# DannielSilva/MM-VQA

Measured on AMD Instinct MI355X. Metric: samples/sec ROCO-MLM pretrain (resnet152+transformer, bs16/GPU, 224^2, seq32), higher is better.
Workload: dtype f32; 1 GPU; pretrain/roco_train.py MLM-only: resnet152 + transformer(4 layers, 12 heads), num_vis 5, hidden 768, vocab 30522, per-GPU batch 16, 224x224, T=32; fwd + log_softmax/NLL + bwd + grad all-reduce + Adam; dropout on, train-mode BN; random-init weights; global_batch=16, seq_len=32, parallelism=dp1

## Files before the change

mm-vqa_amd/csrc/igemm.hip:

```cpp
#include <string>
#include <type_traits>
#include <vector>

#include "kernels.h"

struct FastDiv {
  uint32_t mul, shr, d;
};
struct GemmAux {
  FastDiv ohw, ow;
  int fast;
  int stagger;
  float* part;
  int ldsc;
  int pad0;
  int sk_gx, sk_gy;
  int sk_slots;
  float* sk_part;
  unsigned* sk_cnt;
  int tick;
  int xcd;
};

__device__ __forceinline__ int fdiv(int n, const FastDiv& f) {
// ... 202 lines not shown
          for (int j = 0; j < 4; ++j) {
            double* d = red + (c4 * 4 + j) * 3;
            atomicAdd(d, (double)sa[j]);
            atomicAdd(d + 1, (double)sb[j]);
            if (st2) atomicAdd(d + 2, (double)sc[j]);
          }
        }
        if (colsum) {
#pragma unroll
          for (int j = 0; j < 4; ++j) atomicAdd(&redf[c4 * 4 + j], cs[j]);
        }
      }
      __syncthreads();
      TRACE_EPI(2);
      if (tid < BN && n0 + tid < N) {
        if (st1) {
          const double* d = red + tid * 3;
          const int slot = slot_seed & ((p.stat_slots > 0 ? p.stat_slots : MMVQA_STAT_SLOTS) - 1);
          double* d1 = st1 + ((size_t)slot * N + n0 + tid) * 2;
          atomicAdd(d1, d[0]);
          atomicAdd(d1 + 1, d[1]);
          if (st2) {
            double* d2 = st2 + ((size_t)slot * N + n0 + tid) * 2;
            atomicAdd(d2, d[0]);
            atomicAdd(d2 + 1, d[2]);
          }
        }
        if (colsum) atomicAdd(&colsum[n0 + tid], redf[tid]);
      }
    }
    }
}

template <int BM, int BN, int BK, int KIND, bool NCHW, int KS, int PREC = MMVQA_PREC_F32>
__global__ __launch_bounds__(256 * KS, 2) void igemm_kernel(const GemmParams p, const GemmAux x) {
  constexpr int NT = 256 * KS;
  constexpr int WM = BM / 2, WN = BN / 2, TM = WM / 32, TN = WN / 32;
  constexpr bool F16 = (PREC == MMVQA_PREC_F16);
  static_assert(!F16 || KS == 1, "the f16 family has no 8-wave form");
  constexpr bool PIPE = TM * TN <= 2;
  constexpr int LDK = F16 ? BK + 8 : BK + 4;
  constexpr int KQ = BK / 4;
  constexpr int RSTEP = NT / KQ;
  constexpr int NA = BM / RSTEP, NB = BN / RSTEP;
  constexpr bool A_ROWK = (KIND != KIND_WGRAD);
  constexpr bool B_ROWK = (KIND == KIND_FWD);
  constexpr int LDA_KM = F16 ? km_ld_h(BM) : BM + 4, LDB_KM = F16 ? km_ld_h(BN) : BN + 4;
  constexpr int A_TILE = A_ROWK ? tile_rowk<PREC>(BM, BK) : tile_km<PREC>(BM, BK);
  constexpr int B_TILE = B_ROWK ? tile_rowk<PREC>(BN, BK) : tile_km<PREC>(BN, BK);
  constexpr int A_X4 = BM / 4, A_KSTEP = NT / A_X4, NA_KM = BK / A_KSTEP;
  constexpr int B_X4 = BN / 4, B_KSTEP = NT / B_X4, NB_KM = BK / B_KSTEP;
  constexpr int NAC = A_ROWK ? NA : NA_KM;
  constexpr int NBC = B_ROWK ? NB : NB_KM;

  TRACE_MARK(0);
  TRACE_STALL_DECL
  extern __shared__ __attribute__((aligned(16))) float smem[];
  float* As = smem;
  float* Bs = smem + 2 * A_TILE;
  int* taptab = reinterpret_cast<int*>(smem + 2 * A_TILE + 2 * B_TILE);
  float* ctab = smem + 2 * A_TILE + 2 * B_TILE + MAX_TAPS;

  const int nkt_total = (p.K + BK - 1) / BK;
  __shared__ int sk_last;
  const int tid = threadIdx.x;
  const int lane = tid & 63, wave = (tid >> 6) & 3, ks = tid >> 8;
  const int li = lane & 31, lh = lane >> 5;
  const int wm0 = (wave >> 1) * WM, wn0 = (wave & 1) * WN;
// ... 174 lines not shown
      int tap = 0;
      if (taps > 1) { tap = nn / p.g_Cs; b_kh = tap / p.g_KW; b_kw = tap - b_kh * p.g_KW; }
      b_ci = nn - tap * p.g_Cs;
      if (p.b_pro != PRO_NONE && b_colvalid) { bc0 = ld4(p.b_c0 + b_ci); bc1 = ld4(p.b_c1 + b_ci); }
    } else {
#pragma unroll
      for (int j = 0; j < 4; ++j) {
        int kk = nn + j;
        int tap = kk / p.g_Cs;
        b_cc[j] = kk - tap * p.g_Cs;
        b_dy[j] = tap / p.g_KW; b_dx[j] = tap - b_dy[j] * p.g_KW;
        if (kk >= p.N) b_dy[j] = -(1 << 24);
      }
    }
#pragma unroll
    for (int r = 0; r < NB_KM; ++r) { b_base[r] = k_begin + bkm_k0 + B_KSTEP * r; b_ok0[r] = 1; }
  }

  struct Stage {
    f32x4 ra[NAC], ra2[NAC], rb[NBC], rb2[NBC];
    uint32_t a_ok, b_ok;
    f32x4 ac0, ac1, ac2;
    int tm[NAC];
    int pm[NBC], tmb[NBC];
  };

  f32x16 acc[TM][TN];
#pragma unroll
  for (int i = 0; i < TM; ++i)
#pragma unroll
    for (int j = 0; j < TN; ++j)
#pragma unroll
      for (int e = 0; e < 16; ++e) acc[i][j][e] = 0.f;

  const int adv_tap = BK / p.g_Cs, adv_c = BK - adv_tap * p.g_Cs;

  auto lds_put = [&](float* tile, int e, f32x4 v) __attribute__((always_inline)) {
    if constexpr (F16) *reinterpret_cast<f16x4*>(reinterpret_cast<_Float16*>(tile) + e) = __builtin_convertvector(v, f16x4);
    else *reinterpret_cast<f32x4*>(&tile[e]) = v;
  };

  auto run = [&](auto APRO_T, auto BPRO_T, auto FAST_T, auto LDSC_T) __attribute__((always_inline)) {
    constexpr int APRO = decltype(APRO_T)::value;
    constexpr int BPRO = decltype(BPRO_T)::value;
    constexpr int FAST = decltype(FAST_T)::value;
    constexpr bool LDSC = decltype(LDSC_T)::value;
    constexpr bool A_TWO = (APRO == PRO_DZ);
    constexpr bool A_AFF = (APRO == PRO_AFFINE_RELU || APRO == PRO_AFFINE_SILU || APRO == PRO_SILU_GATE);
    constexpr bool B_AFF = (BPRO == PRO_AFFINE_RELU || BPRO == PRO_AFFINE_SILU || BPRO == PRO_SILU_GATE);

    constexpr int NLP = 1 + NAC + NBC;
    bool lt_kvalid = false;
    int lt_toff = 0;
    int lt_kh[4], lt_kw[4], lt_c[4];
    auto load_piece = [&](Stage& S, int kt, int i) __attribute__((always_inline)) {
      if (i == 0) {
        S.a_ok = 0; S.b_ok = 0;
        if constexpr (A_ROWK && !NCHW) {
          lt_kvalid = a_tap < taps;
          lt_toff = taptab[lt_kvalid ? a_tap : 0];
          if constexpr (A_AFF || A_TWO) {
            const int cc = lt_kvalid ? a_c : 0;
            S.ac0 = ld4(p.a_c0 + cc); S.ac1 = ld4(p.a_c1 + cc);
            if constexpr (APRO == PRO_DZ) S.ac2 = ld4(p.a_c2 + cc);
          }
        }
// ... 332 lines not shown
        }
      } else {
        const int r = c - NAC;
        f32x4 v = S.rb[r];
        if constexpr (KIND == KIND_WGRAD && BPRO == PRO_AFFINE_RELU) {
          const f32x2 lo = __builtin_elementwise_fma(v.xy, bc0.xy, bc1.xy), hi = __builtin_elementwise_fma(v.zw, bc0.zw, bc1.zw);
          if constexpr (FAST == 2) {
            const float lim = __builtin_bit_cast(float, S.tmb[r] & 0x7f800000);
            v[0] = __builtin_amdgcn_fmed3f(lo[0], 0.f, lim); v[1] = __builtin_amdgcn_fmed3f(lo[1], 0.f, lim);
            v[2] = __builtin_amdgcn_fmed3f(hi[0], 0.f, lim); v[3] = __builtin_amdgcn_fmed3f(hi[1], 0.f, lim);
          } else {
            v[0] = fmaxf(lo[0], 0.f); v[1] = fmaxf(lo[1], 0.f); v[2] = fmaxf(hi[0], 0.f); v[3] = fmaxf(hi[1], 0.f);
          }
        }
        if constexpr (B_ROWK) {
          lds_put(bs, (b_r0 + RSTEP * r) * LDK + b_kq, v);
        } else {
          lds_put(bs, (bkm_k0 + B_KSTEP * r) * LDB_KM + bkm_x4 * 4, v);
        }
      }
    };
    auto LP = [&](Stage& S, int kt, int i) __attribute__((always_inline)) {
      if constexpr (FAST != 0) fload_piece(S, i); else load_piece(S, kt, i);
    };
    auto SC = [&](Stage& S, int buf, int kt, int c) __attribute__((always_inline)) {
      if constexpr (FAST != 0) fstore_chunk(S, buf, c); else store_chunk(S, buf, kt, c);
    };
    auto LT = [&](Stage& S, int kt) __attribute__((always_inline)) {
#pragma unroll
      for (int i = 0; i < NLP; ++i) LP(S, kt, i);
    };

    auto read_frags = [&](const float* as, const float* bs, int kg, f32x4 (&fa)[TM], f32x4 (&fb)[TN]) __attribute__((always_inline)) {
#pragma unroll
      for (int i = 0; i < TM; ++i) {
        if constexpr (A_ROWK) {
          fa[i] = *reinterpret_cast<const f32x4*>(&as[(wm0 + i * 32 + li) * LDK + kg * 8 + lh * 4]);
        } else {
#pragma unroll
          for (int j = 0; j < 4; ++j) fa[i][j] = as[(kg * 8 + lh * 4 + j) * LDA_KM + wm0 + i * 32 + li];
        }
      }
#pragma unroll
      for (int i = 0; i < TN; ++i) {
        if constexpr (B_ROWK) {
          fb[i] = *reinterpret_cast<const f32x4*>(&bs[(wn0 + i * 32 + li) * LDK + kg * 8 + lh * 4]);
        } else {
#pragma unroll
          for (int j = 0; j < 4; ++j) fb[i][j] = bs[(kg * 8 + lh * 4 + j) * LDB_KM + wn0 + i * 32 + li];
        }
      }
    };

    constexpr int NC = NAC + NBC;
    constexpr int NKG = BK / 8 / KS;

    TRACE_MARK(1);
    Stage S0, S1;
    S0.a_ok = S0.b_ok = S1.a_ok = S1.b_ok = 0;
    S0.ac0 = S1.ac0 = ac0_i; S0.ac1 = S1.ac1 = ac1_i; S0.ac2 = S1.ac2 = ac2_i;

    if constexpr (FAST == 2 && KIND == KIND_WGRAD) {
#pragma unroll
      for (int r = 0; r < NBC; ++r) { S0.pm[r] = tload(f_voffT[r], 0); S1.pm[r] = tload(f_voffT[r], BK * 4); }
    }
    if (nkt > 0) {
      LT(S0, kt_begin);
      if constexpr (PIPE) LT(S1, kt_begin + 1);
#pragma unroll
      for (int c = 0; c < NC; ++c) SC(S0, 0, kt_begin, c);
      if constexpr (FAST != 0 && PIPE && !F16) f_halo(S0);
    }
    __builtin_amdgcn_s_waitcnt(0x0F70);
    __syncthreads();
    TRACE_MARK(2);

    if constexpr (F16) {
      auto frag = [&](const float* tile, int rowk, int ldkm, int r0, int st) __attribute__((always_inline)) {
        const _Float16* t = reinterpret_cast<const _Float16*>(tile);
        if (rowk) return *reinterpret_cast<const f16x8*>(t + (r0 + li) * LDK + st * 16 + lh * 8);
        const int g = lane >> 4, q = (lane >> 2) & 3, pp = lane & 3;
        const _Float16* b = t + (st * 16 + (g >> 1) * 8 + q) * ldkm + r0 + (g & 1) * 16 + 4 * pp;
        typedef __attribute__((address_space(3))) s16x4 lds_s16x4;
        const f16x4 lo = __builtin_bit_cast(f16x4, __builtin_amdgcn_ds_read_tr16_b64_v4i16((lds_s16x4*)(b)));
        const f16x4 hi = __builtin_bit_cast(f16x4, __builtin_amdgcn_ds_read_tr16_b64_v4i16((lds_s16x4*)(b + 4 * ldkm)));
        return __builtin_shufflevector(lo, hi, 0, 1, 2, 3, 4, 5, 6, 7);
      };
      auto body16 = [&](int t, Stage& Sload, Stage& Sstore) __attribute__((always_inline)) {
        const int buf = t & 1;
        LT(Sload, kt_begin + t + (PIPE ? 2 : 1));
        const float* as = As + buf * A_TILE;
        const float* bs = Bs + buf * B_TILE;
#pragma unroll
        for (int st = 0; st < BK / 16; ++st) {
          f16x8 fa[TM], fb[TN];
#pragma unroll
          for (int i = 0; i < TM; ++i) fa[i] = frag(as, A_ROWK, LDA_KM, wm0 + i * 32, st);
#pragma unroll
          for (int i = 0; i < TN; ++i) fb[i] = frag(bs, B_ROWK, LDB_KM, wn0 + i * 32, st);
#pragma unroll
          for (int a = 0; a < TM; ++a)
#pragma unroll
            for (int b = 0; b < TN; ++b)
              acc[a][b] = __builtin_amdgcn_mfma_f32_32x32x16_f16(fa[a], fb[b], acc[a][b], 0, 0, 0);
        }
#pragma unroll
        for (int c = 0; c < NC; ++c) SC(Sstore, buf ^ 1, kt_begin + t + 1, c);
        __syncthreads();
      };
      if constexpr (PIPE) {
        int t = 0;
        for (; t + 1 < nkt; t += 2) {
          body16(t, S0, S1);
          body16(t + 1, S1, S0);
        }
        if (t < nkt) body16(t, S0, S1);
      } else {
        for (int t = 0; t < nkt; ++t) body16(t, S0, S0);
      }
    } else if constexpr (PIPE) {
      f32x4 fa[2][TM], fb[2][TN];
      read_frags(As, Bs, ks, fa[0], fb[0]);
      constexpr int MPG = 4 * TM * TN;
      constexpr int NS = NKG * MPG;
      constexpr int SB = NS - MPG;
      constexpr int L0 = 1;
      constexpr int LSTR = (NS - 2) / NLP > 0 ? (NS - 2) / NLP : 1;
      constexpr int ST0 = LSTR >= 2 ? L0 + 1 : L0 + NLP;
      constexpr int STR = LSTR >= 2 ? LSTR : ((SB - ST0) / NC > 0 ? (SB - ST0) / NC : 1);
      static_assert(ST0 + (NC - 1) * STR < SB, "load/store pieces do not fit in front of the barrier");
      constexpr int SV = SB - (NS >= 32 ? 5 : 3);
      constexpr int FLS = (SV - 2) / NC > 0 ? (SV - 2) / NC : 1;
      static_assert(2 + (NC - 1) * FLS < SV, "fast load slots must precede the VALU slot");
      static_assert(2 + (NC - 1) * FLS + 1 < NS, "staggered group: advance/halo slot inside the K-tile");
      auto body = [&](auto STG_T, int t, Stage& Sload, Stage& Sstore) __attribute__((always_inline)) {
        constexpr bool STG = decltype(STG_T)::value;
        constexpr int SVX = STG ? 1 : SV;
        const int buf = t & 1;
        const float* as = As + buf * A_TILE;
        const float* bs = Bs + buf * B_TILE;
        static_for<NS>([&](auto SI) __attribute__((always_inline)) {
          constexpr int sl = decltype(SI)::value, kk = sl / MPG, g = sl % MPG;
          constexpr int j = g / (TM * TN), ta = (g % (TM * TN)) / TN, tb = g % TN;
          if constexpr (g == 0) {
            if constexpr (kk + 1 < NKG) {
              read_frags(as, bs, (kk + 1) * KS + ks, fa[(kk + 1) & 1], fb[(kk + 1) & 1]);
            } else {
#ifdef IGEMM_TRACE
              {
                const unsigned long long ta = __builtin_readcyclecounter();
                __builtin_amdgcn_s_waitcnt(0xC07F);
                const unsigned long long tb = __builtin_readcyclecounter();
                __syncthreads();
                const unsigned long long tc = __builtin_readcyclecounter();
                tr_lgkm += tb - ta; tr_bar += tc - tb;
              }
#elif !defined(EXP_NOBAR)
              __syncthreads();
#endif
              read_frags(As + (buf ^ 1) * A_TILE, Bs + (buf ^ 1) * B_TILE, ks, fa[0], fb[0]);
            }
          }
          acc[ta][tb] = __builtin_amdgcn_mfma_f32_32x32x2f32(fa[kk & 1][ta][j], fb[kk & 1][tb][j], acc[ta][tb], 0, 0, 0);
#ifndef EXP_NOLOAD
          if constexpr (FAST != 0) {
            if constexpr (sl == 1) f_scalars(Sload);
            if constexpr (sl >= 2 && (STG || sl < SV) && (sl - 2) % FLS == 0 && (sl - 2) / FLS < NC) f_chunk(Sload, (sl - 2) / FLS);
          } else {
            if constexpr (sl >= L0 && (sl - L0) % LSTR == 0 && (sl - L0) / LSTR < NLP)
              LP(Sload, kt_begin + t + 2, (sl - L0) / LSTR);
          }
#endif
#ifndef EXP_NOSTORE
#ifdef IGEMM_TRACE
          if constexpr (sl == SVX && FAST != 0) {
            constexpr int NLD = (A_ROWK && (A_AFF || A_TWO) ? (APRO == PRO_DZ ? 3 : 2) : 0) + NAC * (A_TWO ? 2 : 1) + NBC;
            const unsigned long long ta = __builtin_readcyclecounter();
            __builtin_amdgcn_s_waitcnt(0x0F70 | (NLD & 15) | ((NLD >> 4) << 14));
            const unsigned long long tb = __builtin_readcyclecounter();
            tr_vm += tb - ta;
          }
#endif
          if constexpr (FAST != 0) {
            if constexpr (sl == SVX) {
#pragma unroll
              for (int c = 0; c < NC; ++c) fstore_chunk(Sstore, buf ^ 1, c);
              if constexpr (!STG) {
                f_advance();
                f_halo(Sstore);
              }
            }
            if constexpr (STG && sl == 2 + (NC - 1) * FLS + 1) {
              f_advance();
              f_halo(Sstore);
            }
          } else {
// ... 68 lines not shown
      } else {
        switch (p.a_pro) {
          case PRO_AFFINE_RELU: run(I1{}, I0{}, G{}, L0{}); break;
          case PRO_AFFINE_SILU: run(I4{}, I0{}, G{}, L0{}); break;
          case PRO_SILU_GATE: run(I5{}, I0{}, G{}, L0{}); break;
          default: run(I0{}, I0{}, G{}, L0{});
        }
      }
    } else if constexpr (KIND == KIND_DGRAD) {
      if (x.fast == 1) {
        if (p.a_pro == PRO_DZ) { if (x.ldsc) run(I2{}, I0{}, F1{}, L1{}); else run(I2{}, I0{}, F1{}, L0{}); }
        else run(I0{}, I0{}, F1{}, L0{});
      } else if (x.fast == 2) {
        if (p.a_pro == PRO_DZ) { if (x.ldsc) run(I2{}, I0{}, F2{}, L1{}); else run(I2{}, I0{}, F2{}, L0{}); }
        else run(I0{}, I0{}, F2{}, L0{});
      } else {
        if (p.a_pro == PRO_DZ) run(I2{}, I0{}, G{}, L0{}); else run(I0{}, I0{}, G{}, L0{});
      }
    } else {
      if (x.fast == 1) {
        if (p.a_pro == PRO_DZ) {
          if (p.b_pro == PRO_AFFINE_RELU) run(I2{}, I1{}, F1{}, L0{}); else run(I2{}, I0{}, F1{}, L0{});
        } else {
          if (p.b_pro == PRO_AFFINE_RELU) run(I0{}, I1{}, F1{}, L0{}); else run(I0{}, I0{}, F1{}, L0{});
        }
      } else if (x.fast == 2) {
        if constexpr (TM * TN == 1) {
          if (p.a_pro == PRO_DZ) {
            if (p.b_pro == PRO_AFFINE_RELU) run(I2{}, I1{}, F2{}, L0{}); else run(I2{}, I0{}, F2{}, L0{});
          } else {
            if (p.b_pro == PRO_AFFINE_RELU) run(I0{}, I1{}, F2{}, L0{}); else run(I0{}, I0{}, F2{}, L0{});
          }
        }
      } else if (p.a_pro == PRO_DZ) {
        switch (p.b_pro) {
          case PRO_AFFINE_RELU: run(I2{}, I1{}, G{}, L0{}); break;
          case PRO_AFFINE_SILU: run(I2{}, I4{}, G{}, L0{}); break;
          case PRO_SILU_GATE: run(I2{}, I5{}, G{}, L0{}); break;
          default: run(I2{}, I0{}, G{}, L0{});
        }
      } else {
        switch (p.b_pro) {
          case PRO_AFFINE_RELU: run(I0{}, I1{}, G{}, L0{}); break;
          case PRO_AFFINE_SILU: run(I0{}, I4{}, G{}, L0{}); break;
          case PRO_SILU_GATE: run(I0{}, I5{}, G{}, L0{}); break;
          default: run(I0{}, I0{}, G{}, L0{});
        }
      }
    }
  }

  TRACE_MARK(3);
  TRACE_STALL_FLUSH();
  constexpr int LDC = BN + 4;
  constexpr int CH = BN / 4;
  constexpr int RP = NT / CH;
  constexpr int NPASS = BM / RP;
  float* ctile = smem;
  if (KS == 1 || ks == 0) {
    static_for<TM * TN * 16>([&](auto I) {
      constexpr int i = decltype(I)::value;
      constexpr int a = i / (TN * 16), b = (i / 16) % TN, e = i % 16;
      ctile[(wm0 + a * 32 + (e & 3) + 8 * (e >> 2) + 4 * lh) * LDC + wn0 + b * 32 + li] = acc[a][b][e];
    });
  }
  __syncthreads();
  if constexpr (KS > 1) {
    if (ks == 1) {
      static_for<TM * TN * 16>([&](auto I) {
        constexpr int i = decltype(I)::value;
        constexpr int a = i / (TN * 16), b = (i / 16) % TN, e = i % 16;
        ctile[(wm0 + a * 32 + (e & 3) + 8 * (e >> 2) + 4 * lh) * LDC + wn0 + b * 32 + li] += acc[a][b][e];
      });
    }
    __syncthreads();
  }

  TRACE_EPI(0);
  const int M = p.M, N = p.N;
  const int c4 = tid % CH, rg = tid / CH;
  const int col = n0 + c4 * 4;
  const bool full = col + 3 < N;
  auto ldv = [&](const float* base, size_t off) __attribute__((always_inline)) {
    f32x4 r = {0, 0, 0, 0};
    if (full && !(off & 3)) r = ld4(base + off);
    else {
#pragma unroll
      for (int j = 0; j < 4; ++j) if (col + j < N) r[j] = base[off + j];
    }
    return r;
  };
  auto stv = [&](float* base, size_t off, f32x4 v) __attribute__((always_inline)) {
    if (full && !(off & 3)) *reinterpret_cast<f32x4*>(base + off) = v;
    else {
#pragma unroll
      for (int j = 0; j < 4; ++j) if (col + j < N) base[off + j] = v[j];
    }
  };

  if (x.tick != 0) {
// ... 150 lines not shown
                                    const size_t off = (size_t)row * N + col;
                                    if (col + 3 < N && !(off & 3)) {
                                      f32x4 t[SK_MAX];
#pragma unroll
                                      for (int s = 0; s < SK_MAX; ++s)
                                        t[s] = s < nsplit ? ld4(part + s * MN + off) : f32x4{0, 0, 0, 0};
#pragma unroll
                                      for (int s = 0; s < SK_MAX; ++s) v += t[s];
                                    } else {
                                      for (int s = 0; s < nsplit; ++s)
#pragma unroll
                                        for (int j = 0; j < 4; ++j)
                                          if (col + j < N) v[j] += part[s * MN + off + j];
                                    }
                                  }
                                  return v;
                                });
}

static FastDiv make_fastdiv(int d) {
  FastDiv f;
  f.d = (uint32_t)d;
  if (d <= 1) { f.mul = 0; f.shr = 0; f.d = 1; return f; }
  int lg = 31;
  while (lg > 0 && !((uint32_t)d >> lg)) --lg;
  if (d & (d - 1)) ++lg;
  const int pw = 31 + lg;
  const uint64_t m = ((1ull << pw) + (uint64_t)d - 1) / (uint64_t)d;
  f.mul = (uint32_t)m;
  f.shr = (uint32_t)(pw - 32);
  return f;
}

template <int BM, int BN, int BK, int KIND, bool NCHW, int KS = 1, int PREC = MMVQA_PREC_F32>
static int launch_cfg(GemmParams p, hipStream_t stream) {
  constexpr bool A_ROWK = (KIND != KIND_WGRAD);
  constexpr bool B_ROWK = (KIND == KIND_FWD);
  constexpr int A_TILE = A_ROWK ? tile_rowk<PREC>(BM, BK) : tile_km<PREC>(BM, BK);
  constexpr int B_TILE = B_ROWK ? tile_rowk<PREC>(BN, BK) : tile_km<PREC>(BN, BK);
  constexpr size_t tile_floats = (size_t)(2 * A_TILE + 2 * B_TILE + MAX_TAPS);
  constexpr size_t epi_floats = (size_t)BM * (BN + 4) + 8 * BN;
  constexpr size_t smem_max = (tile_floats + FOLD_MAX_FLOATS > epi_floats ? tile_floats + FOLD_MAX_FLOATS : epi_floats) * sizeof(float);
  static int attr_dev_mask = 0;
  int dev = 0;
  (void)hipGetDevice(&dev);
  if (!(attr_dev_mask >> (dev & 31) & 1)) {
    HIP_CHECK_RET(hipFuncSetAttribute((const void*)igemm_kernel<BM, BN, BK, KIND, NCHW, KS, PREC>,
                                      hipFuncAttributeMaxDynamicSharedMemorySize, (int)smem_max));
    attr_dev_mask |= 1 << (dev & 31);
  }
  GemmAux x;
  x.ohw = make_fastdiv(p.g_OH * p.g_OW);
  x.ow = make_fastdiv(p.g_OW);
  x.fast = 0;
  static const int stagger_on = getenv("MMVQA_IGEMM_NOSTAGGER") ? 0 : 1;
  x.stagger = stagger_on;
  x.part = (KIND != KIND_WGRAD && !NCHW && p.splitk > 1 && !p.c_atomic) ? p.sk_ws : nullptr;
  if (!NCHW && (p.K % BK == 0 || (KIND == KIND_WGRAD && p.pixmask)) && !p.gate && !getenv("MMVQA_IGEMM_GENERAL")) {
    const int taps = p.g_KH * p.g_KW;
    const double lim = 2147483648.0 - 16777216.0;
    if (KIND != KIND_WGRAD) {
      const bool pro_ok = (KIND == KIND_FWD) ? (p.a_pro == PRO_NONE || p.a_pro == PRO_AFFINE_RELU)
                                             : (p.a_pro == PRO_NONE || p.a_pro == PRO_DZ);
      const double a_bytes = (KIND == KIND_FWD) ? (double)p.M * p.g_stride * p.g_stride * p.a_ld * 4.0 + (double)(p.g_SW + 2) * p.g_KH * p.a_ld * 4.0
                                                : (double)p.M * p.a_ld * 4.0;
      const double b_bytes = (KIND == KIND_FWD) ? (double)p.N * p.b_ld * 4.0 : (double)p.g_Cs * p.b_ld * 4.0;
      if (pro_ok && p.b_pro == PRO_NONE && p.g_Cs % BK == 0 && p.g_stride <= 2 && a_bytes < lim && b_bytes < lim &&
          (KIND == KIND_FWD || p.N % 4 == 0))
        x.fast = (taps > 1 || (KIND == KIND_DGRAD && p.g_stride > 1)) ? 2 : 1;
    } else {
      const bool pro_ok = (p.a_pro == PRO_NONE || p.a_pro == PRO_DZ) && (p.b_pro == PRO_NONE || p.b_pro == PRO_AFFINE_RELU);
      if (pro_ok && taps == 1 && p.K % BK == 0 && p.g_stride == 1 && p.g_pad == 0 && p.M % 4 == 0 && p.N % 4 == 0 &&
          (double)p.K * p.a_ld * 4.0 < lim && (double)p.K * p.b_ld * 4.0 < lim)
        x.fast = 1;
      else if (pro_ok && taps > 1 && taps <= 32 && p.pixmask && p.g_stride == 1 && p.g_OH == p.g_SH && p.g_OW == p.g_SW &&
               2 * p.g_pad == p.g_KH - 1 && p.g_KH == p.g_KW && BM == 64 && BN == 64 && p.g_Cs % BN == 0 && p.M % 4 == 0 &&
               (double)p.K * p.a_ld * 4.0 < lim && (double)(p.K + (double)p.g_SW * p.g_KH) * p.b_ld * 4.0 < lim)
        x.fast = 2;
    }
  }
// ... 11 lines not shown
      const int C = A_ROWK ? p.g_Cs : p.M;
      if (!f.publish || !f.out0 || !f.out1 || !f.out2)
        return mmvqa_set_error(MMVQA_ERR_ARG, "igemm: this launch cannot fold its BatchNorm coefficients in the kernel and has nowhere to publish them");
      if (f.bwd)
        TRY_RET(k_bn_coef_bwd(stream, f.stat, C, f.count, f.gamma, f.mean, f.invstd, 1, f.out0, f.out1, f.out2, f.dgamma, f.dbeta));
      else
        TRY_RET(k_bn_coef_fwd_keep(stream, f.stat, C, f.count, f.eps, f.gamma, f.beta, f.run_mean, f.run_var, f.nbt, f.keep,
                                   f.reps, 1, f.out0, f.out1, f.out2, f.out3));
      p.a_c0 = f.out0; p.a_c1 = f.out1; p.a_c2 = f.out2;
      p.a_fold.stat = nullptr;
    }
  }
  const size_t smem = ((tile_floats + fold_floats > epi_floats ? tile_floats + fold_floats : epi_floats)) * sizeof(float);
  dim3 grid((p.N + BN - 1) / BN, (p.M + BM - 1) / BM, p.splitk);
  x.pad0 = 0; x.sk_gx = (int)grid.x; x.sk_gy = (int)grid.y; x.sk_slots = 0; x.sk_part = nullptr; x.sk_cnt = nullptr; x.tick = 0;
  static const bool finish_form = getenv("MMVQA_SK_FINISH") != nullptr;
  if (x.part && !finish_form && p.sk_cnt && p.splitk <= SK_PART_MAX && p.epi_mode == EPI_PLAIN) {
    const long long tiles = (long long)grid.x * grid.y;
    if (tiles <= p.sk_cnt_n && tiles * p.splitk * (long long)(BM * BN) <= p.sk_ws_floats) {
      x.tick = 1; x.part = nullptr; x.sk_slots = p.splitk; x.sk_part = p.sk_ws; x.sk_cnt = p.sk_cnt;
    }
  }
  static const int xcd_on = getenv("MMVQA_IGEMM_NOXCD") ? 0 : 1;
  const long nwg = (long)grid.x * grid.y * grid.z;
  x.xcd = 0;
  if (xcd_on && nwg >= 32 && !NCHW) {
    double a_bytes, b_bytes;
    if (KIND == KIND_WGRAD) { a_bytes = (double)p.K * p.M * (p.a_pro == PRO_DZ ? 2 : 1); b_bytes = (double)p.K * p.g_Cs; }
    else if (KIND == KIND_FWD) { a_bytes = (double)p.M * p.g_stride * p.g_stride * p.g_Cs; b_bytes = (double)p.N * p.K; }
    else { a_bytes = (double)p.M * p.g_Cs * (p.a_pro == PRO_DZ ? 2 : 1); b_bytes = (double)p.N * p.K; }
    x.xcd = (b_bytes > a_bytes && x.sk_gy > 1) ? 2 : (x.sk_gx > 1 ? 1 : 0);
  }
  if (getenv("MMVQA_IGEMM_LOG"))
    fprintf(stderr, "igemm kind %d fast %d tile %dx%dx%d ks %d M %d N %d K %d Cs %d taps %d stride %d apro %d bpro %d splitk %d fold %d tick %d prec %s\n", KIND, x.fast,
            BM, BN, BK, KS, p.M, p.N, p.K, p.g_Cs, p.g_KH * p.g_KW, p.g_stride, p.a_pro, p.b_pro, p.splitk, x.ldsc, x.tick,
            PREC == MMVQA_PREC_F16 ? "f16" : "f32");
  hipLaunchKernelGGL((igemm_kernel<BM, BN, BK, KIND, NCHW, KS, PREC>), grid, dim3(256 * KS), smem, stream, p, x);
  KERNEL_CHECK_RET();
  if (x.part) {
    hipLaunchKernelGGL(splitk_finish_kernel, dim3((p.N + 63) / 64, (p.M + 63) / 64), dim3(256), 0, stream, p, x.part,
                       p.splitk);
    KERNEL_CHECK_RET();
  }
  return MMVQA_OK;
}

static inline int cdiv(int a, int b) { return (a + b - 1) / b; }

static bool sk_eligible(const GemmParams& p, int kind) {
  return kind != KIND_WGRAD && p.sk_ws && p.sk_ws_floats > 0 && p.epi_mode == EPI_PLAIN && !p.c_atomic;
}

static thread_local IgemmTuner* g_tuner = nullptr;
void mmvqa_set_tuner(IgemmTuner* t) { g_tuner = t; }
static thread_local int g_prec = MMVQA_PREC_F32;
void mmvqa_set_igemm_precision(int prec) { g_prec = prec; }

static std::string tune_key(const GemmParams& p, int kind, int nchw) {
  char buf[176];
  snprintf(buf, sizeof(buf), "%d,%d,%d,%d,%d,%d,%d,%d,%d,%d,%d,%d,%d,%d,%d,%d", p.reserved0, kind, nchw, p.M, p.N, p.K,
           p.g_KH * p.g_KW, p.g_stride, p.g_Cs, p.a_pro, p.b_pro, p.epi_mode, p.act | (p.dact << 4),
           (p.stat1 ? 1 : 0) | (p.stat2 ? 2 : 0) | (p.Mk ? 4 : 0) | (p.R ? 8 : 0) | (p.Cpre ? 16 : 0) |
               (p.colsum ? 32 : 0) | (p.bias ? 64 : 0) | (p.sk_ws ? 128 : 0) | (p.a_fold.stat ? 256 : 0) | (p.sk_cnt ? 512 : 0),
           p.c_atomic, p.splitk);
  return buf;
}

static int launch_one(GemmParams p, int kind, int nchw, int tile, hipStream_t stream);

static int validate_desc(const GemmParams& p, int kind, int nchw) {
#define BAD(...) return mmvqa_set_error(MMVQA_ERR_ARG, "igemm: " __VA_ARGS__)
  if (kind < KIND_FWD || kind > KIND_WGRAD) BAD("unknown kind %d", kind);
  if (p.reserved0 != MMVQA_PREC_F32 && p.reserved0 != MMVQA_PREC_F16) BAD("unknown operand precision %d (reserved0)", p.reserved0);
  if (p.reserved1 != 0) BAD("reserved1=%d must be 0 (the persistent form was removed)", p.reserved1);
  if (p.reserved0 == MMVQA_PREC_F16 && (p.a_pro == PRO_AFFINE_SILU || p.a_pro == PRO_SILU_GATE || p.b_pro == PRO_AFFINE_SILU ||
                                        p.b_pro == PRO_SILU_GATE || p.gate))
    BAD("the f16 operand family has no SiLU / gate prologues (a_pro %d, b_pro %d)", p.a_pro, p.b_pro);
  if (!p.A || !p.B) BAD("operand pointer is null (A=%p B=%p)", (const void*)p.A, (const void*)p.B);
  if (!p.C && p.epi_mode != EPI_TAP_FWD) BAD("output pointer is null");
  const int KH = p.g_KH > 0 ? p.g_KH : 1, KW = p.g_KH > 0 ? p.g_KW : 1;
  const long taps = (long)KH * KW;
  if (KW <= 0 || p.g_Cs <= 0 || (p.g_KH > 0 && (p.g_stride <= 0 || p.g_pad < 0))) BAD("bad geometry (KH=%d KW=%d Cs=%d stride=%d pad=%d)", p.g_KH, p.g_KW, p.g_Cs, p.g_stride, p.g_pad);
  if (p.g_OH <= 0 || p.g_OW <= 0 || p.g_SH <= 0 || p.g_SW <= 0) BAD("bad image dims (SH=%d SW=%d OH=%d OW=%d)", p.g_SH, p.g_SW, p.g_OH, p.g_OW);
  const long ohw = (long)p.g_OH * p.g_OW;
  if (kind == KIND_WGRAD) {
    if ((long)p.N != taps * p.g_Cs) BAD("wgrad: N=%d != taps*Cs=%ld", p.N, taps * p.g_Cs);
    if (p.K % ohw) BAD("wgrad: K=%d is not a multiple of OH*OW=%ld", p.K, ohw);
    if (p.a_ld < p.M || (!nchw && p.b_ld < p.g_Cs) || p.c_ld < p.N) BAD("wgrad: leading dimension too small (a_ld=%d M=%d b_ld=%d Cs=%d c_ld=%d N=%d)", p.a_ld, p.M, p.b_ld, p.g_Cs, p.c_ld, p.N);
  } else {
    if ((long)p.K != taps * p.g_Cs) BAD("K=%d != taps*Cs=%ld", p.K, taps * p.g_Cs);
    if (p.M % ohw) BAD("M=%d is not a multiple of OH*OW=%ld", p.M, ohw);
    if (!nchw && p.a_ld < p.g_Cs) BAD("a_ld=%d < Cs=%d", p.a_ld, p.g_Cs);
    if (kind == KIND_FWD && p.b_ld < p.K) BAD("fwd: b_ld=%d < K=%d", p.b_ld, p.K);
    if (kind == KIND_DGRAD && ((long)p.b_ld < (taps - 1) * p.b_tapstride + p.N)) BAD("dgrad: b_ld=%d < (taps-1)*tapstride+N", p.b_ld);
    if (p.epi_mode == EPI_PLAIN && p.c_ld < p.N) BAD("c_ld=%d < N=%d", p.c_ld, p.N);
  }
  if (p.a_fold.stat) {
    const mmvqa_bn_fold& f = p.a_fold;
    if (f.slots <= 0 || f.slots > MMVQA_STAT_SLOTS || (f.slots & (f.slots - 1))) BAD("a_fold.slots=%d is not a power of two <= %d", f.slots, MMVQA_STAT_SLOTS);
    if (!(f.count > 0.0) || !f.gamma) BAD("a_fold without count / gamma");
    if (f.bwd ? (p.a_pro != PRO_DZ || !f.mean || !f.invstd) : (p.a_pro != PRO_AFFINE_RELU || !f.beta)) BAD("a_fold.bwd=%d does not match A prologue %d (or mean / invstd / beta missing)", f.bwd, p.a_pro);
    if (f.publish && (!f.out0 || !f.out1 || !f.out2 || (f.bwd ? (!f.dgamma || !f.dbeta) : !f.out3))) BAD("a_fold.publish without output arrays");
    if (nchw && kind != KIND_WGRAD) BAD("a_fold: not for the NCHW stem forward");
  } else if (p.a_pro != PRO_NONE && (!p.a_c0 || !p.a_c1)) BAD("A prologue %d without coefficients", p.a_pro);
  if (p.a_pro == PRO_DZ && (!p.A2 || (!p.a_c2 && !p.a_fold.stat))) BAD("BatchNorm-backward prologue without A2 / c2");
  if (p.stat_slots < 0 || p.stat_slots > MMVQA_STAT_SLOTS || (p.stat_slots & (p.stat_slots - 1))) BAD("stat_slots=%d is not a power of two <= %d", p.stat_slots, MMVQA_STAT_SLOTS);
  if (p.b_pro != PRO_NONE && (!p.b_c0 || !p.b_c1)) BAD("B prologue %d without coefficients", p.b_pro);
  if ((p.a_pro == PRO_SILU_GATE || p.b_pro == PRO_SILU_GATE) && (!p.gate || p.gate_hw <= 0)) BAD("gate prologue without gate tensor");
  if (p.dact != ACT_NONE && !p.Pre) BAD("act' epilogue without the saved pre-activation");
  if (p.stat_bwd && p.stat1 && (!p.Z1 || !p.mean1 || !p.invstd1)) BAD("backward statistics without Z1 / mean / invstd");
  if (p.stat2 && (!p.stat1 || !p.Z2 || !p.mean2 || !p.invstd2)) BAD("second statistics set incomplete");
  if (p.epi_mode == EPI_TAP_FWD && (!p.tap_out || p.tap_HW <= 0)) BAD("tap epilogue without output / HW");
  if (p.epi_mode == EPI_TAP_BWD && (!p.tap_dv || p.tap_HW <= 0)) BAD("tap backward epilogue without dv / HW");
  if (p.Mk && p.mk_ld < p.N) BAD("mask tensor leading dimension %d < N=%d", p.mk_ld, p.N);
  if (p.R && p.r_ld < p.N) BAD("residual leading dimension %d < N=%d", p.r_ld, p.N);
  if (p.drop_p < 0.f || p.drop_p >= 1.f) BAD("dropout p=%g outside [0,1)", (double)p.drop_p);
#undef BAD
  return MMVQA_OK;
}

int mmvqa_launch_igemm(GemmParams p, int kind, int nchw, int tile, hipStream_t stream) {
  if (p.M <= 0 || p.N <= 0 || p.K <= 0) return MMVQA_OK;
  if (p.reserved0 == MMVQA_PREC_F32) p.reserved0 = g_prec;
  if (int r = validate_desc(p, kind, nchw)) return r;
  if (tile != 0 || nchw || !g_tuner) return launch_one(p, kind, nchw, tile, stream);
  const std::string key = tune_key(p, kind, nchw);
  auto it = g_tuner->table.find(key);
  if (it == g_tuner->table.end()) {
    if (!g_tuner->tuning) return launch_one(p, kind, nchw, 0, stream);
    struct Cand { int tile, splitk; };
    std::vector<Cand> cands;
    const int tiles_f[] = {1, 2, 3, 4, 5, 6}, tiles_w[] = {1, 2, 3, 4, 5, 6};
    if (kind == KIND_WGRAD && p.splitk <= 0) {
      for (int t : tiles_w) for (int sk : {0, 1, 2, 3, 4, 6, 8, 12, 16}) cands.push_back({t, sk});
    } else if (kind == KIND_WGRAD) {
      for (int t : tiles_w) cands.push_back({t, p.splitk});
    } else if (sk_eligible(p, kind) && p.splitk <= 0 && (long)cdiv(p.M, 64) * cdiv(p.N, 64) <= 320) {
      for (int t : {3, 5, 6}) for (int sk : {1, 2, 3, 4, 6, 8}) cands.push_back({t, sk});
      for (int t : {1, 2, 4}) cands.push_back({t, 1});
    } else {
      for (int t : tiles_f) cands.push_back({t, p.splitk});
    }
    hipEvent_t e0, e1;
    HIP_CHECK_RET(hipEventCreate(&e0));
    HIP_CHECK_RET(hipEventCreate(&e1));
    float best = 1e30f, best_single = 1e30f;
    Cand bc = cands[0], bc_single = cands[0];
    const bool sk_partial = kind != KIND_WGRAD && sk_eligible(p, kind) && p.splitk <= 0;
    static const float sk_gain = getenv("MMVQA_SK_GAIN") ? (float)atof(getenv("MMVQA_SK_GAIN")) : (getenv("MMVQA_SK_FINISH") ? 0.85f : 0.92f);
    for (const Cand& c : cands) {
      GemmParams q = p;
      q.splitk = c.splitk;
      int r = launch_one(q, kind, nchw, c.tile, stream);
      if (r != MMVQA_OK) continue;
      static const int tune_reps = getenv("MMVQA_TUNE_REPS") ? atoi(getenv("MMVQA_TUNE_REPS")) : 3;
      float ms = 1e30f;
      for (int rep = 0; rep < (tune_reps > 0 ? tune_reps : 1); ++rep) {
        HIP_CHECK_RET(hipEventRecord(e0, stream));
        for (int i = 0; i < 3; ++i) launch_one(q, kind, nchw, c.tile, stream);
        HIP_CHECK_RET(hipEventRecord(e1, stream));
        HIP_CHECK_RET(hipEventSynchronize(e1));
        float t = 0.f;
        HIP_CHECK_RET(hipEventElapsedTime(&t, e0, e1));
        if (t < ms) ms = t;
      }
      if (ms < best) { best = ms; bc = c; }
      if (c.splitk <= 1 && ms < best_single) { best_single = ms; bc_single = c; }
    }
    if (sk_partial && bc.splitk > 1 && best_single < 1e29f && best > sk_gain * best_single) { bc = bc_single; best = best_single; }
    hipEventDestroy(e0);
    hipEventDestroy(e1);
    it = g_tuner->table.emplace(key, IgemmChoice{bc.tile, bc.splitk}).first;
  }
  p.splitk = it->second.splitk;
  return launch_one(p, kind, nchw, it->second.tile, stream);
}

static int launch_one(GemmParams p, int kind, int nchw, int tile, hipStream_t stream) {
  if (p.M <= 0 || p.N <= 0 || p.K <= 0) return MMVQA_OK;
  if (p.g_KH <= 0) { p.g_KH = p.g_KW = 1; p.g_stride = 1; p.g_pad = 0; }
  if (!nchw && p.g_KH * p.g_KW > MAX_TAPS)
    return mmvqa_set_error(MMVQA_ERR_ARG, "igemm: at most %d taps in the NHWC gather", MAX_TAPS);
  if ((double)p.M * p.a_ld > 2.0e9 && kind != KIND_WGRAD)
    return mmvqa_set_error(MMVQA_ERR_ARG, "igemm: operand A exceeds 2^31 elements");
  if (tile == 0) {
    long t128 = (long)cdiv(p.M, 128) * cdiv(p.N, 128);
    long t12864 = (long)cdiv(p.M, 128) * cdiv(p.N, 64);
    if (t128 >= 384) tile = 1;
    else if (t12864 >= 384 || (p.N <= 64 && p.M >= 4096)) tile = 2;
    else tile = 3;
    if (tile == 3 && kind != KIND_WGRAD && (long)cdiv(p.M, 64) * cdiv(p.N, 64) < 400 && p.K >= 512) tile = 5;
  }
  if (nchw) tile = (kind == KIND_FWD) ? 2 : 3;
  const bool f16 = p.reserved0 == MMVQA_PREC_F16;
  if (f16 && tile == 5) tile = 3;
  const int bm = (tile == 1 || tile == 2) ? 128 : 64;
  const int bn = (tile == 1 || tile == 4) ? 128 : 64;
  const int bk = ((tile == 3 || tile == 5) && !nchw) ? 64 : 32;
  const int nkt = cdiv(p.K, bk);
  if (p.splitk <= 0) {
    p.splitk = 1;
    if (kind == KIND_WGRAD) {
      long tiles = (long)cdiv(p.M, bm) * cdiv(p.N, bn);
      int want = (int)((512 + tiles - 1) / tiles);
      int per = bk == 64 ? 2 : 4;
      int maxs = nkt / per > 0 ? nkt / per : 1;
      p.splitk = want < maxs ? want : maxs;
      if (p.splitk < 1) p.splitk = 1;
      if (p.splitk > 1) p.c_atomic = 1;
    } else if (!nchw && sk_eligible(p, kind)) {
      const long tiles = (long)cdiv(p.M, bm) * cdiv(p.N, bn);
      if (tiles <= 128 && p.K >= 1024) {
        int want = (int)((256 + tiles - 1) / tiles);
        const int maxs = p.K / 256;
        if (want > maxs) want = maxs;
        if (want > 8) want = 8;
        if (want > 1) p.splitk = want;
      }
    }
  }
  if (kind != KIND_WGRAD && !nchw && p.splitk > 1 && !p.c_atomic) {
    if (!sk_eligible(p, kind))
      return mmvqa_set_error(MMVQA_ERR_ARG, "igemm: split-K needs an accumulating epilogue or a scratch (sk_ws)");
    const long long cap = p.sk_ws_floats / ((long long)p.M * p.N);
    if (p.splitk > cap) p.splitk = (int)(cap < 1 ? 1 : cap);
    if (p.splitk > SK_MAX) p.splitk = SK_MAX;
  }
  p.ktiles_per_split = cdiv(nkt, p.splitk);
  p.splitk = cdiv(nkt, p.ktiles_per_split);
  if (p.splitk > 1 && !p.c_atomic && !(kind != KIND_WGRAD && !nchw && sk_eligible(p, kind)))
    return mmvqa_set_error(MMVQA_ERR_ARG, "igemm: split-K needs an accumulating epilogue");
#define GO(BM_, BN_, BK_)                                                                                          \
  do {                                                                                                             \
    if (f16) {                                                                                                     \
      if (kind == KIND_FWD) return launch_cfg<BM_, BN_, BK_, KIND_FWD, false, 1, MMVQA_PREC_F16>(p, stream);     \
      if (kind == KIND_DGRAD) return launch_cfg<BM_, BN_, BK_, KIND_DGRAD, false, 1, MMVQA_PREC_F16>(p, stream); \
      return launch_cfg<BM_, BN_, BK_, KIND_WGRAD, false, 1, MMVQA_PREC_F16>(p, stream);                         \
    }                                                                                                              \
    if (kind == KIND_FWD) return launch_cfg<BM_, BN_, BK_, KIND_FWD, false>(p, stream);                            \
    if (kind == KIND_DGRAD) return launch_cfg<BM_, BN_, BK_, KIND_DGRAD, false>(p, stream);                        \
    return launch_cfg<BM_, BN_, BK_, KIND_WGRAD, false>(p, stream);                                                \
  } while (0)
  if (nchw && f16) {
    if (kind == KIND_FWD) return launch_cfg<128, 64, 32, KIND_FWD, true, 1, MMVQA_PREC_F16>(p, stream);
    if (kind == KIND_WGRAD) return launch_cfg<64, 64, 32, KIND_WGRAD, true, 1, MMVQA_PREC_F16>(p, stream);
    return mmvqa_set_error(MMVQA_ERR_ARG, "igemm: no NCHW dgrad");
  }
  if (nchw) {
    if (kind == KIND_FWD) return launch_cfg<128, 64, 32, KIND_FWD, true>(p, stream);
    if (kind == KIND_WGRAD) return launch_cfg<64, 64, 32, KIND_WGRAD, true>(p, stream);
    return mmvqa_set_error(MMVQA_ERR_ARG, "igemm: no NCHW dgrad");
  }
  switch (tile) {
    case 1: GO(128, 128, 32);
    case 2: GO(128, 64, 32);
    case 4: GO(64, 128, 32);
    case 6: GO(64, 64, 32);
    case 5:
      if (kind == KIND_FWD) return launch_cfg<64, 64, 64, KIND_FWD, false, 2>(p, stream);
      if (kind == KIND_DGRAD) return launch_cfg<64, 64, 64, KIND_DGRAD, false, 2>(p, stream);
      return launch_cfg<64, 64, 64, KIND_WGRAD, false, 2>(p, stream);
    default: GO(64, 64, 64);
  }
#undef GO
  return MMVQA_OK;
}
```

Before: 661.1 samples/s.

## Add k-sliced weight-gradient igemm variant using 16x16x4 MFMA with per-wave K split

```diff
diff --git a/mm-vqa_amd/csrc/igemm.hip b/mm-vqa_amd/csrc/igemm.hip
--- a/mm-vqa_amd/csrc/igemm.hip
+++ b/mm-vqa_amd/csrc/igemm.hip
@@ -258,8 +258,16 @@
     }
 }
 
-template <int BM, int BN, int BK, int KIND, bool NCHW, int KS, int PREC = MMVQA_PREC_F32>
+constexpr int KIND_WGRAD_KSL = 3;
+template <bool ON> struct KsliceAcc { f32x4 v[4][4]; };
+template <> struct KsliceAcc<false> {};
+template <int BM, int BN, int BK, int KIND_T, bool NCHW, int KS, int PREC = MMVQA_PREC_F32>
 __global__ __launch_bounds__(256 * KS, 2) void igemm_kernel(const GemmParams p, const GemmAux x) {
+  constexpr bool KSL = (KIND_T == KIND_WGRAD_KSL);
+  constexpr int KIND = KSL ? (int)KIND_WGRAD : KIND_T;
+  constexpr int NW = 4 * KS;
+  static_assert(!KSL || (BM == 64 && BN == 64 && !NCHW && PREC == MMVQA_PREC_F32 && BK % (4 * NW) == 0 && (BK / 4 / NW) % 2 == 0),
+                "k-sliced weight gradient: 64x64 tiles, fp32 family, an even number of k-steps per wave and K-tile");
   constexpr int NT = 256 * KS;
   constexpr int WM = BM / 2, WN = BN / 2, TM = WM / 32, TN = WN / 32;
   constexpr bool F16 = (PREC == MMVQA_PREC_F16);
@@ -500,6 +508,13 @@
     for (int j = 0; j < TN; ++j)
 #pragma unroll
       for (int e = 0; e < 16; ++e) acc[i][j][e] = 0.f;
+  KsliceAcc<KSL> kacc;
+  if constexpr (KSL) {
+#pragma unroll
+    for (int i = 0; i < 4; ++i)
+#pragma unroll
+      for (int j = 0; j < 4; ++j) kacc.v[i][j] = f32x4{0, 0, 0, 0};
+  }
 
   const int adv_tap = BK / p.g_Cs, adv_c = BK - adv_tap * p.g_Cs;
 
@@ -898,6 +913,12 @@
     };
 
     auto read_frags = [&](const float* as, const float* bs, int kg, f32x4 (&fa)[TM], f32x4 (&fb)[TN]) __attribute__((always_inline)) {
+      if constexpr (KSL) {
+        const int kc = lane & 15, kq = lane >> 4;
+        fa[0] = *reinterpret_cast<const f32x4*>(&as[(kg * 4 + kq) * LDA_KM + kc * 4]);
+        fb[0] = *reinterpret_cast<const f32x4*>(&bs[(kg * 4 + kq) * LDB_KM + kc * 4]);
+        return;
+      }
 #pragma unroll
       for (int i = 0; i < TM; ++i) {
         if constexpr (A_ROWK) {
@@ -919,7 +940,9 @@
     };
 
     constexpr int NC = NAC + NBC;
-    constexpr int NKG = BK / 8 / KS;
+    constexpr int NKG = KSL ? BK / 4 / NW : BK / 8 / KS;
+    const int kg0 = KSL ? (tid >> 6) : ks;
+    constexpr int KGS = KSL ? NW : KS;
 
     TRACE_MARK(1);
     Stage S0, S1;
@@ -986,16 +1009,17 @@
       }
     } else if constexpr (PIPE) {
       f32x4 fa[2][TM], fb[2][TN];
-      read_frags(As, Bs, ks, fa[0], fb[0]);
-      constexpr int MPG = 4 * TM * TN;
+      read_frags(As, Bs, kg0, fa[0], fb[0]);
+      constexpr int MPG = KSL ? 16 : 4 * TM * TN;
       constexpr int NS = NKG * MPG;
-      constexpr int SB = NS - MPG;
+      constexpr int GB = KSL ? MPG - 6 : 0;
+      constexpr int SB = NS - MPG + GB;
       constexpr int L0 = 1;
       constexpr int LSTR = (NS - 2) / NLP > 0 ? (NS - 2) / NLP : 1;
       constexpr int ST0 = LSTR >= 2 ? L0 + 1 : L0 + NLP;
       constexpr int STR = LSTR >= 2 ? LSTR : ((SB - ST0) / NC > 0 ? (SB - ST0) / NC : 1);
       static_assert(ST0 + (NC - 1) * STR < SB, "load/store pieces do not fit in front of the barrier");
-      constexpr int SV = SB - (NS >= 32 ? 5 : 3);
+      constexpr int SV = SB - (KSL ? 10 : NS >= 32 ? 5 : 3);
       constexpr int FLS = (SV - 2) / NC > 0 ? (SV - 2) / NC : 1;
       static_assert(2 + (NC - 1) * FLS < SV, "fast load slots must precede the VALU slot");
       static_assert(2 + (NC - 1) * FLS + 1 < NS, "staggered group: advance/halo slot inside the K-tile");
@@ -1008,10 +1032,9 @@
         static_for<NS>([&](auto SI) __attribute__((always_inline)) {
           constexpr int sl = decltype(SI)::value, kk = sl / MPG, g = sl % MPG;
           constexpr int j = g / (TM * TN), ta = (g % (TM * TN)) / TN, tb = g % TN;
-          if constexpr (g == 0) {
-            if constexpr (kk + 1 < NKG) {
-              read_frags(as, bs, (kk + 1) * KS + ks, fa[(kk + 1) & 1], fb[(kk + 1) & 1]);
-            } else {
+          if constexpr (g == 0 && kk + 1 < NKG) read_frags(as, bs, (kk + 1) * KGS + kg0, fa[(kk + 1) & 1], fb[(kk + 1) & 1]);
+          if constexpr (g == GB) {
+            if constexpr (kk + 1 == NKG) {
 #ifdef IGEMM_TRACE
               {
                 const unsigned long long ta = __builtin_readcyclecounter();
@@ -1024,10 +1047,13 @@
 #elif !defined(EXP_NOBAR)
               __syncthreads();
 #endif
-              read_frags(As + (buf ^ 1) * A_TILE, Bs + (buf ^ 1) * B_TILE, ks, fa[0], fb[0]);
+              read_frags(As + (buf ^ 1) * A_TILE, Bs + (buf ^ 1) * B_TILE, kg0, fa[0], fb[0]);
             }
           }
-          acc[ta][tb] = __builtin_amdgcn_mfma_f32_32x32x2f32(fa[kk & 1][ta][j], fb[kk & 1][tb][j], acc[ta][tb], 0, 0, 0);
+          if constexpr (KSL)
+            kacc.v[g / 4][g % 4] = __builtin_amdgcn_mfma_f32_16x16x4f32(fa[kk & 1][0][g / 4], fb[kk & 1][0][g % 4], kacc.v[g / 4][g % 4], 0, 0, 0);
+          else
+            acc[ta][tb] = __builtin_amdgcn_mfma_f32_32x32x2f32(fa[kk & 1][ta][j], fb[kk & 1][tb][j], acc[ta][tb], 0, 0, 0);
 #ifndef EXP_NOLOAD
           if constexpr (FAST != 0) {
             if constexpr (sl == 1) f_scalars(Sload);
@@ -1162,6 +1188,12 @@
             if (p.b_pro == PRO_AFFINE_RELU) run(I0{}, I1{}, F2{}, L0{}); else run(I0{}, I0{}, F2{}, L0{});
           }
         }
+      } else if constexpr (KSL) {
+        if (p.a_pro == PRO_DZ) {
+          if (p.b_pro == PRO_AFFINE_RELU) run(I2{}, I1{}, G{}, L0{}); else run(I2{}, I0{}, G{}, L0{});
+        } else {
+          if (p.b_pro == PRO_AFFINE_RELU) run(I0{}, I1{}, G{}, L0{}); else run(I0{}, I0{}, G{}, L0{});
+        }
       } else if (p.a_pro == PRO_DZ) {
         switch (p.b_pro) {
           case PRO_AFFINE_RELU: run(I2{}, I1{}, G{}, L0{}); break;
@@ -1187,7 +1219,35 @@
   constexpr int RP = NT / CH;
   constexpr int NPASS = BM / RP;
   float* ctile = smem;
-  if (KS == 1 || ks == 0) {
+  if constexpr (KSL) {
+    constexpr int CT = BM * LDC;
+    constexpr int NREG0 = (2 * A_TILE + 2 * B_TILE) / CT, NREG = NREG0 < NW ? NREG0 : NW;
+    static_assert(NREG >= 1 && NW % NREG == 0, "staged partial tiles must fit the tile buffers");
+    const int kw = tid >> 6, kc = lane & 15, kq = lane >> 4;
+    float* reg = smem + (kw % NREG) * CT + (16 * kq) * LDC + 4 * kc;
+    static_for<NW / NREG>([&](auto R) {
+      constexpr int r = decltype(R)::value;
+      if (kw / NREG == r) {
+        static_for<16>([&](auto I) {
+          constexpr int i = decltype(I)::value / 4, e = decltype(I)::value % 4;
+          f32x4 v = {kacc.v[i][0][e], kacc.v[i][1][e], kacc.v[i][2][e], kacc.v[i][3][e]};
+          f32x4* q = reinterpret_cast<f32x4*>(reg + (4 * e + i) * LDC);
+          if constexpr (r > 0) v += *q;
+          *q = v;
+        });
+      }
+      __syncthreads();
+    });
+    if constexpr (NREG > 1) {
+      for (int i = tid; i < BM * CH; i += NT) {
+        const int off = (i / CH) * LDC + (i % CH) * 4;
+        f32x4 v = *reinterpret_cast<const f32x4*>(&ctile[off]);
+#pragma unroll
+        for (int g = 1; g < NREG; ++g) v += *reinterpret_cast<const f32x4*>(&ctile[g * CT + off]);
+        *reinterpret_cast<f32x4*>(&ctile[off]) = v;
+      }
+    }
+  } else if (KS == 1 || ks == 0) {
     static_for<TM * TN * 16>([&](auto I) {
       constexpr int i = decltype(I)::value;
       constexpr int a = i / (TN * 16), b = (i / 16) % TN, e = i % 16;
@@ -1195,7 +1255,7 @@
     });
   }
   __syncthreads();
-  if constexpr (KS > 1) {
+  if constexpr (KS > 1 && !KSL) {
     if (ks == 1) {
       static_for<TM * TN * 16>([&](auto I) {
         constexpr int i = decltype(I)::value;
@@ -1412,8 +1472,10 @@
   return f;
 }
 
-template <int BM, int BN, int BK, int KIND, bool NCHW, int KS = 1, int PREC = MMVQA_PREC_F32>
+template <int BM, int BN, int BK, int KIND, bool NCHW, int KS = 1, int PREC = MMVQA_PREC_F32, bool KSL = false>
 static int launch_cfg(GemmParams p, hipStream_t stream) {
+  static_assert(!KSL || KIND == KIND_WGRAD, "the k-sliced mapping is a weight-gradient form");
+  constexpr int KIND_T = KSL ? KIND_WGRAD_KSL : KIND;
   constexpr bool A_ROWK = (KIND != KIND_WGRAD);
   constexpr bool B_ROWK = (KIND == KIND_FWD);
   constexpr int A_TILE = A_ROWK ? tile_rowk<PREC>(BM, BK) : tile_km<PREC>(BM, BK);
@@ -1425,7 +1487,7 @@
   int dev = 0;
   (void)hipGetDevice(&dev);
   if (!(attr_dev_mask >> (dev & 31) & 1)) {
-    HIP_CHECK_RET(hipFuncSetAttribute((const void*)igemm_kernel<BM, BN, BK, KIND, NCHW, KS, PREC>,
+    HIP_CHECK_RET(hipFuncSetAttribute((const void*)igemm_kernel<BM, BN, BK, KIND_T, NCHW, KS, PREC>,
                                       hipFuncAttributeMaxDynamicSharedMemorySize, (int)smem_max));
     attr_dev_mask |= 1 << (dev & 31);
   }
@@ -1503,10 +1565,10 @@
     x.xcd = (b_bytes > a_bytes && x.sk_gy > 1) ? 2 : (x.sk_gx > 1 ? 1 : 0);
   }
   if (getenv("MMVQA_IGEMM_LOG"))
-    fprintf(stderr, "igemm kind %d fast %d tile %dx%dx%d ks %d M %d N %d K %d Cs %d taps %d stride %d apro %d bpro %d splitk %d fold %d tick %d prec %s\n", KIND, x.fast,
+    fprintf(stderr, "igemm kind %d%s fast %d tile %dx%dx%d ks %d M %d N %d K %d Cs %d taps %d stride %d apro %d bpro %d splitk %d fold %d tick %d prec %s\n", KIND, KSL ? " (k-sliced)" : "", x.fast,
             BM, BN, BK, KS, p.M, p.N, p.K, p.g_Cs, p.g_KH * p.g_KW, p.g_stride, p.a_pro, p.b_pro, p.splitk, x.ldsc, x.tick,
             PREC == MMVQA_PREC_F16 ? "f16" : "f32");
-  hipLaunchKernelGGL((igemm_kernel<BM, BN, BK, KIND, NCHW, KS, PREC>), grid, dim3(256 * KS), smem, stream, p, x);
+  hipLaunchKernelGGL((igemm_kernel<BM, BN, BK, KIND_T, NCHW, KS, PREC>), grid, dim3(256 * KS), smem, stream, p, x);
   KERNEL_CHECK_RET();
   if (x.part) {
     hipLaunchKernelGGL(splitk_finish_kernel, dim3((p.N + 63) / 64, (p.M + 63) / 64), dim3(256), 0, stream, p, x.part,
@@ -1538,6 +1600,11 @@
 }
 
 static int launch_one(GemmParams p, int kind, int nchw, int tile, hipStream_t stream);
+
+static bool wgrad_kslice_on() {
+  static const bool on = !getenv("MMVQA_WGRAD_KSLICE_OFF");
+  return on;
+}
 
 static int validate_desc(const GemmParams& p, int kind, int nchw) {
 #define BAD(...) return mmvqa_set_error(MMVQA_ERR_ARG, "igemm: " __VA_ARGS__)
@@ -1601,7 +1668,9 @@
     if (!g_tuner->tuning) return launch_one(p, kind, nchw, 0, stream);
     struct Cand { int tile, splitk; };
     std::vector<Cand> cands;
-    const int tiles_f[] = {1, 2, 3, 4, 5, 6}, tiles_w[] = {1, 2, 3, 4, 5, 6};
+    const int tiles_f[] = {1, 2, 3, 4, 5, 6};
+    std::vector<int> tiles_w = {1, 2, 3, 4, 5, 6};
+    if (kind == KIND_WGRAD && p.reserved0 == MMVQA_PREC_F32 && wgrad_kslice_on()) tiles_w.insert(tiles_w.end(), {7, 8, 9});
     if (kind == KIND_WGRAD && p.splitk <= 0) {
       for (int t : tiles_w) for (int sk : {0, 1, 2, 3, 4, 6, 8, 12, 16}) cands.push_back({t, sk});
     } else if (kind == KIND_WGRAD) {
@@ -1654,6 +1723,7 @@
     return mmvqa_set_error(MMVQA_ERR_ARG, "igemm: at most %d taps in the NHWC gather", MAX_TAPS);
   if ((double)p.M * p.a_ld > 2.0e9 && kind != KIND_WGRAD)
     return mmvqa_set_error(MMVQA_ERR_ARG, "igemm: operand A exceeds 2^31 elements");
+  const bool auto_tile = tile == 0;
   if (tile == 0) {
     long t128 = (long)cdiv(p.M, 128) * cdiv(p.N, 128);
     long t12864 = (long)cdiv(p.M, 128) * cdiv(p.N, 64);
@@ -1662,12 +1732,18 @@
     else tile = 3;
     if (tile == 3 && kind != KIND_WGRAD && (long)cdiv(p.M, 64) * cdiv(p.N, 64) < 400 && p.K >= 512) tile = 5;
   }
+  const bool f16 = p.reserved0 == MMVQA_PREC_F16;
+  if (tile >= 7 && tile <= 9 && (kind != KIND_WGRAD || f16))
+    return mmvqa_set_error(MMVQA_ERR_ARG, "igemm: tile %d is a weight-gradient form of the fp32 family", tile);
+  const bool ksl_pro_ok = p.b_pro == PRO_NONE || p.b_pro == PRO_AFFINE_RELU;
+  if (tile >= 7 && tile <= 9 && !ksl_pro_ok)
+    return mmvqa_set_error(MMVQA_ERR_ARG, "igemm: tile %d has no SiLU / gate prologue (b_pro %d)", tile, p.b_pro);
+  if (auto_tile && tile == 3 && kind == KIND_WGRAD && !f16 && ksl_pro_ok && wgrad_kslice_on()) tile = 7;
   if (nchw) tile = (kind == KIND_FWD) ? 2 : 3;
-  const bool f16 = p.reserved0 == MMVQA_PREC_F16;
   if (f16 && tile == 5) tile = 3;
   const int bm = (tile == 1 || tile == 2) ? 128 : 64;
   const int bn = (tile == 1 || tile == 4) ? 128 : 64;
-  const int bk = ((tile == 3 || tile == 5) && !nchw) ? 64 : 32;
+  const int bk = ((tile == 3 || tile == 5 || tile == 7 || tile == 8) && !nchw) ? 64 : 32;
   const int nkt = cdiv(p.K, bk);
   if (p.splitk <= 0) {
     p.splitk = 1;
@@ -1727,6 +1803,9 @@
     case 2: GO(128, 64, 32);
     case 4: GO(64, 128, 32);
     case 6: GO(64, 64, 32);
+    case 7: return launch_cfg<64, 64, 64, KIND_WGRAD, false, 1, MMVQA_PREC_F32, true>(p, stream);
+    case 8: return launch_cfg<64, 64, 64, KIND_WGRAD, false, 2, MMVQA_PREC_F32, true>(p, stream);
+    case 9: return launch_cfg<64, 64, 32, KIND_WGRAD, false, 1, MMVQA_PREC_F32, true>(p, stream);
     case 5:
       if (kind == KIND_FWD) return launch_cfg<64, 64, 64, KIND_FWD, false, 2>(p, stream);
       if (kind == KIND_DGRAD) return launch_cfg<64, 64, 64, KIND_DGRAD, false, 2>(p, stream);
```

Measured after the change: 652.9 samples/s. 1.2% lower.
